# kuldeepbrd1/graspLDM

Hardware: AMD Instinct MI355X
Metric: grasps/sec whole-node (1024-pt cloud, 100 DDIM steps) (higher is better)
Workload: dtype f32 (GEMMs as split-f16 x3 partial products on the f16 matrix pipe, f32 accumulation; GroupNorm / LayerNorm / attention / scheduler in f32); 1 GPU; LDM mode, 256 synthetic 1024-pt clouds per GPU x 20 grasps, 100 DDIM steps: BASELINE.json configs[2] per GPU (configs[3] = this per-GPU workload on 8 GPUs); experiment=fpc, clouds_per_gpu=256, grasps_per_cloud=20, points=1024, ddim_steps=100, encoder=PVCNNEncoder (shipped fpc config), parallelism=cloud-sharded x1, weights=synthetic recipe seed 0, streams=3

## Files before the change

### graspldm_amd/_lib.py

```python
import ctypes
import os

_PKG = os.path.dirname(os.path.abspath(__file__))
LIB_PATH = os.environ.get("GLDM_LIB") or os.path.join(_PKG, "libgldm_hip.so")

ABI_VERSION = 14


class GldmError(RuntimeError):
    pass


_lib = None

_ll = ctypes.c_longlong
_ull = ctypes.c_ulonglong
_vp, _i, _f = ctypes.c_void_p, ctypes.c_int, ctypes.c_float

_SIGNATURES = {
    "gldm_ball_query": [_vp, _vp, _i, _i, _i, _f, _i, _vp, _vp],
    "gldm_grouping_forward": [_vp, _vp, _i, _i, _i, _i, _i, _vp, _vp],
    "gldm_gather_features_forward": [_vp, _vp, _i, _i, _i, _i, _vp, _vp],
    "gldm_furthest_point_sampling": [_vp, _i, _i, _i, _vp, _vp],
    "gldm_three_nn_interpolate_forward": [_vp, _vp, _vp, _i, _i, _i, _i, _vp, _vp, _vp, _vp],
    "gldm_avg_voxelize_forward": [_vp, _vp, _i, _i, _i, _i, _vp, _vp, _vp, _vp],
    "gldm_trilinear_devoxelize_forward": [_vp, _vp, _i, _i, _i, _i, _i, _vp, _vp, _vp, _vp],
    "gldm_voxel_coords": [_vp, _i, _i, _i, _i, _f, _vp, _vp, _vp],
    "gldm_farthest_points_euclid": [_vp, _i, _i, _i, _vp, _vp],
    "gldm_normalize_cloud": [_vp, _i, _i, _f, _f, _f, _f, _f, _f, _vp, _vp, _vp],
    "gldm_gather_points": [_vp, _vp, _i, _i, _i, _vp, _vp],
    "gldm_sa_group": [_vp, _vp, _vp, _i, _i, _i, _i, _f, _i, _vp, _vp, _vp],
    "gldm_r1d_cond_embed": [_vp, _vp, _vp, _i, _i, _i, _i, _vp, _vp],
    "gldm_denoise": [_vp, _vp, _vp, _vp, _i, _vp, _i, _vp, _vp, _i, _i, _i, _vp, _vp, _vp, _vp, _vp, _vp],
    "gldm_denoise_rng": [_vp, _vp, _vp, _vp, _i, _vp, _i, _vp, _i, _i, _vp, _ull, _ll, _vp, _vp, _vp, _vp],
    "gldm_step_noise_rng": [_ull, _ll, _i, _i, _i, _vp, _vp],
    "gldm_decode": [_vp, _vp, _vp, _i, _vp, _i, _vp, _vp, _vp, _vp],
    "gldm_pose_epilogue": [_vp, _vp, _vp, _vp, _i, _i, _i, _vp, _vp, _vp, _vp],
    "gldm_encode": [_vp, _vp, _vp, _i, _vp, _i, _vp, _f, _f, _i, _vp, _vp, _vp, _vp, _vp],
    "gldm_pose_prologue": [_vp, _vp, _vp, _vp, _i, _i, _i, _vp, _vp],
    "gldm_conv3d_k3": [_vp, _vp, _vp, _i, _i, _i, _i, _vp, _vp, _vp],
    "gldm_conv3d_k3_cl": [_vp, _vp, _vp, _i, _i, _i, _i, _vp, _vp, _vp],
    "gldm_conv3d_k3_generic": [_vp, _vp, _vp, _i, _i, _i, _i, _vp, _vp, _vp],
    "gldm_conv3d_k3_f16x2": [_vp, _vp, _vp, _i, _i, _i, _i, _vp, _vp, _vp],
    "gldm_conv3d_k3_f16x2_gn": [_vp, _vp, _vp, _vp, _i, _i, _i, _i, _vp, _vp, _i, _vp],
    "gldm_groupnorm_coef": [_vp, _vp, _vp, _i, _i, _i, _i, _f, _vp, _vp],
    "gldm_gn_swish_chan_sum": [_vp, _vp, _i, _i, _i, _vp, _vp],
    "gldm_gn_swish_chan_sum_cl": [_vp, _vp, _i, _i, _i, _vp, _vp],
    "gldm_se_gate_parts": [_vp, _i, _vp, _vp, _i, _i, _i, _i, _i, _vp, _vp],
    "gldm_groupnorm_swish": [_vp, _vp, _vp, _vp, _i, _i, _i, _i, _f, _vp, _vp],
    "gldm_se_gate": [_vp, _vp, _vp, _i, _i, _i, _i, _i, _vp, _vp],
    "gldm_bias_act": [_vp, _vp, _i, _i, ctypes.c_longlong, _i, _vp],
    "gldm_devoxelize_fused": [_vp, _vp, _vp, _vp, _i, _i, _i, _i, _vp, _vp],
    "gldm_devoxelize_gn_fused": [_vp, _vp, _vp, _vp, _vp, _i, _i, _i, _i, _vp, _vp],
    "gldm_devoxelize_gn_cl_fused": [_vp, _vp, _vp, _vp, _vp, _i, _i, _i, _i, _vp, _vp],
    "gldm_pointwise_mlp": [_vp, _vp, _vp, _i, _i, _i, _i, _i, _vp, _vp, _i, _vp, _vp, _vp],
    "gldm_pointwise_mlp2": [_vp, _vp, _vp, _i, _vp, _vp, _i, _i, _i, _i, _vp, _vp, _i, _vp, _vp, _vp],
    "gldm_pointwise_small": [_vp, _vp, _vp, _i, _i, _i, ctypes.c_longlong, _i, _vp, _vp],
    "gldm_pointwise_any": [_vp, _vp, _vp, _i, _i, _i, ctypes.c_longlong, _i, _vp, _vp],
    "gldm_linear_rows": [_vp, _vp, _vp, _i, _i, _i, _vp, _vp],
    "gldm_pointwise_mlp_f16x2": [_vp, _vp, _vp, _i, _i, _i, _i, _i, _vp, _vp, _i, _vp, _vp, _vp],
    "gldm_row_max": [_vp, _ll, _i, _vp, _vp],
    "gldm_pointwise_mlp_f16x2_pm": [_vp, _vp, _vp, _i, _i, _i, _i, _i, _vp, _vp],
    "gldm_pointwise_mlp_f16x2_add": [_vp, _vp, _vp, _vp, _ll, _ll, _ll, _i, _i, _i, _i, _i, _vp, _vp],
    "gldm_pointwise_mlp2_f16x2": [_vp, _vp, _vp, _i, _vp, _vp, _i, _i, _i, _i, _vp, _vp, _i, _vp, _vp, _vp, _vp],
    "gldm_point_attention": [_vp, _vp, _vp, _i, _i, _i, _i, _vp, _ll, _vp, _vp],
    "gldm_point_attention_workspace_bytes": [_i, _i, _i],
    "gldm_groupnorm_swish_points": [_vp, _vp, _vp, _vp, _i, _i, _i, _i, _f, _vp, _vp],
# ... 76 lines not shown
```

### graspldm_amd/csrc/voxel_conv.hip

```cpp
#include <hip/hip_runtime.h>
#include <stdint.h>
#include <stdio.h>
#include <stdlib.h>

#include "gldm.h"
#include "wstream.h"
#include "devstate.h"

#define GLDM_API extern "C" __attribute__((visibility("default")))

namespace {

using f32x4 = __attribute__((ext_vector_type(4))) float;
typedef __attribute__((address_space(3))) float lds_f;

#ifdef GLDM_DEBUG_KNOBS
__device__ long long g_c3_stamp[32];
#define GLDM_C3_STAMP(i) \
  do { if (blockIdx.x == 5 && blockIdx.y == (gridDim.y >> 1) && threadIdx.x == 0) g_c3_stamp[i] = (long long)__builtin_readcyclecounter(); } while (0)
#else
#define GLDM_C3_STAMP(i) do {} while (0)
#endif

template <int CTRL>
__device__ __forceinline__ float dpp_mov(float x) {
  return __int_as_float(__builtin_amdgcn_update_dpp(0, __float_as_int(x), CTRL, 0xf, 0xf, false));
}
__device__ __forceinline__ float row16_sum(float x) {
  x += dpp_mov<0xB1>(x);
  x += dpp_mov<0x4E>(x);
  x += dpp_mov<0x141>(x);
  x += dpp_mov<0x140>(x);
  return x;
}

constexpr int kConvThreads = 256;
constexpr int kBrick = 4;

__host__ __device__ constexpr bool brick_vec4(int r) { return r <= 24; }
__host__ __device__ constexpr int brick_zp(int r) { return brick_vec4(r) ? r + 8 : r + 2; }
__host__ __device__ constexpr int brick_row_stride(int r) {
  return ((6 * 6 * brick_zp(r) + 31) / 32 * 32 + 16) - 32 >= 6 * 6 * brick_zp(r) ? (6 * 6 * brick_zp(r) + 31) / 32 * 32 - 16
                                                                                 : (6 * 6 * brick_zp(r) + 31) / 32 * 32 + 16;
}

template <int MT, int NTW, int JN>
__global__ __launch_bounds__(kConvThreads, 2) void conv3d_k3_kernel(const float *__restrict__ x,
                                                                    const float *__restrict__ wp,
                                                                    const float *__restrict__ bias, int cin, int cout,
                                                                    int r_arg, float *__restrict__ y,
                                                                    float *__restrict__ partial, int cout_total, int co0,
                                                                    int out_cl) {
  constexpr int r = 4 * NTW;
  (void)r_arg;
  extern __shared__ float lds[];
  __builtin_amdgcn_s_setprio(3);
  GLDM_C3_STAMP(0);
  const int tid = threadIdx.x, wave = tid >> 6, lane = tid & 63;
  const int col = lane & 15, kq = lane >> 4;
  const int bpr = r / kBrick;
// ... 200 lines not shown
#pragma unroll
    for (int mi = 0; mi < MT; ++mi)
#pragma unroll
      for (int q = 0; q < 4; ++q) {
        const int co = 16 * mi + 4 * kq + q;
        if (co < cout) {
#pragma unroll
          for (int ni = 0; ni < NTW; ++ni) y[(size_t)co * r3 + gvox[ni]] = acc[mi][ni][q];
        }
      }
  }
  GLDM_C3_STAMP(21);
}

typedef __attribute__((ext_vector_type(8))) _Float16 c3_f16x8;
typedef __attribute__((ext_vector_type(2))) _Float16 c3_f16x2;
typedef __attribute__((ext_vector_type(2))) float c3_f32x2;
typedef __attribute__((ext_vector_type(4))) unsigned c3_u32x4;
constexpr int kC3Split = 2;

__device__ __forceinline__ void c3_split(const float (&x)[8], c3_u32x4 (&pl)[kC3Split]) {
#pragma unroll
  for (int q = 0; q < 4; ++q) {
    const float a = x[2 * q], b = x[2 * q + 1];
    const c3_f16x2 h = __builtin_convertvector(c3_f32x2{a, b}, c3_f16x2);
    const float ra = __builtin_fmaf((float)h[0], -1.0f, a), rb = __builtin_fmaf((float)h[1], -1.0f, b);
    pl[0][q] = __builtin_bit_cast(unsigned, h);
    pl[1][q] = __builtin_bit_cast(unsigned, __builtin_convertvector(c3_f32x2{ra, rb}, c3_f16x2));
  }
}
__device__ __forceinline__ f32x4 c3_mfma(const c3_u32x4 &a, const c3_u32x4 &b, const f32x4 &c) {
  return __builtin_amdgcn_mfma_f32_16x16x32_f16(__builtin_bit_cast(c3_f16x8, a), __builtin_bit_cast(c3_f16x8, b), c, 0, 0, 0);
}
__device__ __forceinline__ f32x4 c3_mfma3(const c3_u32x4 (&a)[kC3Split], const c3_u32x4 (&b)[kC3Split], f32x4 acc) {
  acc = c3_mfma(a[0], b[1], acc);
  acc = c3_mfma(a[1], b[0], acc);
  return c3_mfma(a[0], b[0], acc);
}

constexpr int kPairs = 14;

__device__ __forceinline__ float c3_range_pow2(float m) {
  int e = (int)((__float_as_uint(m) >> 23) & 0xffu) - 127;
  if ((e >= -8 && e < 14) || e < -100 || e > 100) return 1.0f;
  e = e < -40 ? -40 : e;
  return __uint_as_float((unsigned)(e - 13 + 127) << 23);
}
__device__ __forceinline__ float c3_pow2_inv(float s) { return __uint_as_float((254u << 23) - __float_as_uint(s)); }
__device__ __forceinline__ float c3_wave_max(float x) {
#pragma unroll
  for (int off = 32; off >= 1; off >>= 1) x = fmaxf(x, __shfl_xor(x, off, 64));
  return x;
}

template <int MT, int R, int ZB, int WAVES, bool ACT = false>
__global__ __launch_bounds__(64 * WAVES, (ZB * 16 / WAVES / 16 >= 6) ? 1 : 2) void conv3d_k3_pl_kernel(const float *__restrict__ x,
                                                                                      const float *__restrict__ wp3,
                                                                                      const float *__restrict__ bias, int cin,
                                                                                      int cout, float *__restrict__ y,
                                                                                      float *__restrict__ partial,
                                                                                      const float *__restrict__ in_coef,
                                                                                      int out_cl) {
  constexpr int r = R, NTW = ZB / WAVES, kThreads = 64 * WAVES, kZParts = R / ZB;
  constexpr int GM = MT % 3 == 0 ? 3 : (MT % 4 == 0 ? 4 : (MT % 2 == 0 ? 2 : 1));
  constexpr int GN = NTW % 3 == 0 ? 3 : (NTW % 2 == 0 ? 2 : 1);
  static_assert(R % ZB == 0 && ZB % WAVES == 0, "whole n-tiles per wave");
  constexpr int MG = MT / GM, NG = NTW / GN;
  constexpr int zp = ZB + 2, nvox = 36 * zp, r3 = r * r * r;
  constexpr int hs = (nvox + 15) & ~15;
  constexpr int kItems = 2 * nvox, kRounds = (kItems + kThreads - 1) / kThreads;
  constexpr bool kDB = R == 24 && ZB == 24;
  constexpr bool kRanged = !ACT;
  extern __shared__ float lds[];
  GLDM_C3_STAMP(0);
  __builtin_amdgcn_s_setprio(3);
  const int tid = threadIdx.x, wave = tid >> 6, lane = tid & 63;
  const int col = lane & 15, kq = lane >> 4;
  const int bpr = r / kBrick;
  const int bxy = blockIdx.x / kZParts, bz0 = (blockIdx.x % kZParts) * ZB;
  const int bx0 = (bxy / bpr) * kBrick, by0 = (bxy % bpr) * kBrick;
  const int b = blockIdx.y;
  const int cblocks = (cin + 15) >> 4, kblocks = kPairs * cblocks;
  x += (size_t)b * cin * r3;
  y += (size_t)b * cout * r3;
  const WStream wv(wp3, lane);
  typedef __attribute__((address_space(3))) c3_u32x4 lds_c4;
  constexpr int kSet = kC3Split * 2 * hs;
  lds_c4 *pl0 = (lds_c4 *)lds;

  int vb[NTW];
#pragma unroll
  for (int ni = 0; ni < NTW; ++ni) {
    const int o = 16 * (wave * NTW + ni) + col;
    const int iz = o % ZB, ixy = o / ZB, ix = ixy >> 2, iy = ixy & 3;
    vb[ni] = (ix * 6 + iy) * zp + iz + (kq & 1) * hs;
  }
  f32x4 acc[MT][NTW];
#pragma unroll
  for (int mi = 0; mi < MT; ++mi) {
    f32x4 bvv;
#pragma unroll
    for (int q = 0; q < 4; ++q) bvv[q] = bias[16 * mi + 4 * kq + q];
#pragma unroll
    for (int ni = 0; ni < NTW; ++ni) acc[mi][ni] = bvv;
  }
  int s_lds[kRounds], s_glb[kRounds];
#pragma unroll
  for (int q = 0; q < kRounds; ++q) {
    const int it = tid + q * kThreads;
    s_lds[q] = -1;
    s_glb[q] = -1;
    if (it < kItems) {
      const int h = it / nvox, v = it - h * nvox;
      const int ixy = v / zp, izp = v - ixy * zp;
      const int gx = bx0 + ixy / 6 - 1, gy = by0 + ixy % 6 - 1, gz = bz0 + izp - 1;
      s_lds[q] = h * hs + v;
      if ((unsigned)gx < (unsigned)r && (unsigned)gy < (unsigned)r && (unsigned)gz < (unsigned)r)
        s_glb[q] = (gx * r + gy) * r + gz + 8 * h * r3;
    }
  }
  {
    const c3_u32x4 z4 = c3_u32x4{0u, 0u, 0u, 0u};
#pragma unroll
    for (int q = 0; q < kRounds; ++q)
      if (s_lds[q] >= 0 && s_glb[q] < 0) {
#pragma unroll
        for (int p3 = 0; p3 < kC3Split; ++p3) {
          pl0[p3 * 2 * hs + s_lds[q]] = z4;
          if constexpr (kDB) pl0[kSet + p3 * 2 * hs + s_lds[q]] = z4;
        }
      }
  }
  float stg[kRounds][8];
  auto stage_load = [&](int cb) {
    const float *xc = x + (size_t)(cb * 16) * r3;
#pragma unroll
    for (int q = 0; q < kRounds; ++q) {
      const int g0 = s_glb[q] >= 0 ? s_glb[q] : 0;
#pragma unroll
      for (int j = 0; j < 8; ++j) stg[q][j] = xc[(size_t)j * r3 + g0];
    }
  };
  float *s_coef = lds + (kDB ? 2 : 1) * kSet * 4;
  if constexpr (ACT) {
    for (int i = tid; i < 2 * cin; i += kThreads) s_coef[i] = in_coef[(size_t)b * cin * 2 + i];
  }
  unsigned s_run_u = 0x3f800000u;
  float *rng = s_coef;
  auto stage_store = [&](int cb) {
    lds_c4 *pl = pl0 + (kDB ? (cb & 1) * kSet : 0);
#pragma unroll
    for (int q = 0; q < kRounds; ++q)
      if (s_glb[q] >= 0) {
        if constexpr (kRanged) {
          const float inv_run = __uint_as_float((254u << 23) - s_run_u);
#pragma unroll
          for (int j = 0; j < 8; ++j) stg[q][j] *= inv_run;
        }
        if constexpr (ACT) {
          const int h = (tid + q * kThreads) / nvox;
          const f32x4 *cf = reinterpret_cast<const f32x4 *>(s_coef + 2 * (16 * cb + 8 * h));
#pragma unroll
          for (int j2 = 0; j2 < 4; ++j2) {
// ... 122 lines not shown
      const int co = 16 * mi + 4 * kq + q;
      float s = 0.f, s2 = 0.f;
#pragma unroll
      for (int ni = 0; ni < NTW; ++ni) {
        const float v = acc[mi][ni][q];
        s += v;
        s2 += v * v;
      }
      s = row16_sum(s);
      s2 = row16_sum(s2);
      if (col == 0) {
        s_part[(wave * MT * 16 + co) * 2] = s;
        s_part[(wave * MT * 16 + co) * 2 + 1] = s2;
      }
    }
  }
  __syncthreads();
  if (tid < cout) {
    float s = 0.f, s2 = 0.f;
    for (int w = 0; w < WAVES; ++w) {
      s += s_part[(w * MT * 16 + tid) * 2];
      s2 += s_part[(w * MT * 16 + tid) * 2 + 1];
    }
    float *p = partial + (((size_t)b * (gridDim.x / kZParts) + bxy) * cout + tid) * 2;
    if constexpr (kZParts == 1) {
      p[0] = s;
      p[1] = s2;
    } else {
      atomicAdd(p, s);
      atomicAdd(p + 1, s2);
    }
  }
  int gvox[NTW];
  {
    int lane_o = lane;
    asm volatile("" : "+v"(lane_o));
#pragma unroll
    for (int ni = 0; ni < NTW; ++ni) {
      const int o = 16 * (wave * NTW + ni) + (lane_o & 15);
      const int iz = o % ZB, ixy = o / ZB, ix = ixy >> 2, iy = ixy & 3;
      gvox[ni] = ((bx0 + ix) * r + by0 + iy) * r + bz0 + iz;
    }
  }
  if (out_cl) {
#pragma unroll
    for (int ni = 0; ni < NTW; ++ni)
#pragma unroll
      for (int mi = 0; mi < MT; ++mi)
        *reinterpret_cast<f32x4 *>(y + (size_t)gvox[ni] * cout + 16 * mi + 4 * kq) = acc[mi][ni];
  } else {
#pragma unroll
    for (int mi = 0; mi < MT; ++mi)
#pragma unroll
      for (int q = 0; q < 4; ++q) {
        const int co = 16 * mi + 4 * kq + q;
#pragma unroll
        for (int ni = 0; ni < NTW; ++ni) y[(size_t)co * r3 + gvox[ni]] = acc[mi][ni][q];
      }
  }
  GLDM_C3_STAMP(21);
}

template <int MT, int R, int CIN, int WAVES>
__global__ __launch_bounds__(64 * WAVES, 4) void conv3d_k3_fewch_sp_kernel(const float *__restrict__ x,
                                                                           const float *__restrict__ wp3,
                                                                           const float *__restrict__ bias,
                                                                           float *__restrict__ y,
                                                                           float *__restrict__ partial) {
  constexpr int r = R, NTW = R / WAVES, kThreads = 64 * WAVES, zp = R + 2, nvox = 36 * zp, r3 = r * r * r;
  static_assert(R % WAVES == 0, "whole n-tiles per wave");
  constexpr int K = 27 * CIN, KB = (K + 31) / 32, cout = 16 * MT;
  constexpr int cs = nvox + ((nvox & 31) == 0 ? 8 : 0);
  extern __shared__ float lds[];
  const int tid = threadIdx.x, wave = tid >> 6, lane = tid & 63;
  const int col = lane & 15, g = lane >> 4;
  const int bpr = r / kBrick;
  const int bx0 = (blockIdx.x / bpr) * kBrick, by0 = (blockIdx.x % bpr) * kBrick;
  const int b = blockIdx.y;
  x += (size_t)b * CIN * r3;
  y += (size_t)b * cout * r3;
  float mx = 0.f;
  for (int i = tid; i < CIN * nvox; i += kThreads) {
    const int ci = i / nvox, v = i - ci * nvox;
    const int ixy = v / zp, izp = v - ixy * zp;
    const int gx = bx0 + ixy / 6 - 1, gy = by0 + ixy % 6 - 1, gz = izp - 1;
    float val = 0.f;
    if ((unsigned)gx < (unsigned)r && (unsigned)gy < (unsigned)r && (unsigned)gz < (unsigned)r)
      val = x[(size_t)ci * r3 + (gx * r + gy) * r + gz];
    lds[ci * cs + v] = val;
    mx = fmaxf(mx, fabsf(val));
  }
  float *rng = lds + CIN * cs;
  mx = c3_wave_max(mx);
  if (lane == 0) rng[wave] = mx;
  int vb[NTW], gvox[NTW];
#pragma unroll
  for (int ni = 0; ni < NTW; ++ni) {
    const int o = 16 * (wave * NTW + ni) + col;
    const int iz = o % r, ixy = o / r, ix = ixy >> 2, iy = ixy & 3;
    vb[ni] = (ix * 6 + iy) * zp + iz;
    gvox[ni] = ((bx0 + ix) * r + by0 + iy) * r + iz;
// ... 62 lines not shown
      const int co = 16 * mi + 4 * g + q;
      float s = 0.f, s2 = 0.f;
#pragma unroll
      for (int ni = 0; ni < NTW; ++ni) {
        const float v = acc[mi][ni][q];
        s += v;
        s2 += v * v;
      }
      s = row16_sum(s);
      s2 = row16_sum(s2);
      if (col == 0) {
        s_part[(wave * MT * 16 + co) * 2] = s;
        s_part[(wave * MT * 16 + co) * 2 + 1] = s2;
      }
    }
  }
  __syncthreads();
  if (tid < cout) {
    float s = 0.f, s2 = 0.f;
    for (int w = 0; w < WAVES; ++w) {
      s += s_part[(w * MT * 16 + tid) * 2];
      s2 += s_part[(w * MT * 16 + tid) * 2 + 1];
    }
    float *p = partial + (((size_t)b * gridDim.x + blockIdx.x) * cout + tid) * 2;
    p[0] = s;
    p[1] = s2;
  }
#pragma unroll
  for (int mi = 0; mi < MT; ++mi)
#pragma unroll
    for (int q = 0; q < 4; ++q) {
      const int co = 16 * mi + 4 * g + q;
#pragma unroll
      for (int ni = 0; ni < NTW; ++ni) y[(size_t)co * r3 + gvox[ni]] = acc[mi][ni][q];
    }
}

__global__ __launch_bounds__(512) void groupnorm_swish_kernel(float *__restrict__ y, const float *__restrict__ partial,
                                                              const float *__restrict__ gamma,
                                                              const float *__restrict__ beta, int c, int r3,
                                                              int nbricks, int groups, float eps,
                                                              float *__restrict__ chan_sum) {
  __shared__ double s_stat[2];
  __shared__ float s_red[8];
  const int g = blockIdx.x, b = blockIdx.y, cpg = c / groups;
  const int tid = threadIdx.x;
  if (tid < 64) {
    double s = 0.0, s2 = 0.0;
    for (int i = tid; i < nbricks * cpg; i += 64) {
      const int br = i / cpg, ch = g * cpg + i % cpg;
      const float *p = partial + (((size_t)b * nbricks + br) * c + ch) * 2;
      s += (double)p[0];
      s2 += (double)p[1];
    }
    for (int off = 32; off >= 1; off >>= 1) {
      s += __shfl_xor(s, off, 64);
      s2 += __shfl_xor(s2, off, 64);
    }
// ... 487 lines not shown
  GLDM_CONV_CASE(2, 4);
  GLDM_CONV_CASE(4, 2);
  GLDM_CONV_CASE(1, 4);
  GLDM_CONV_CASE(2, 2);
  GLDM_CONV_CASE(4, 1);
  GLDM_CONV_CASE(8, 1);
#undef GLDM_CONV_CASE
  if (mt == 4 && ntw == 8) return launch_conv_halves<2, 8>(x, w_packed, bias, b, cin, cout, r, y, partial, s, out_cl);
  if (mt == 16 && ntw == 2) return launch_conv_halves<8, 2>(x, w_packed, bias, b, cin, cout, r, y, partial, s, out_cl);
  if (mt == 8 && ntw == 4) return launch_conv_halves<4, 4>(x, w_packed, bias, b, cin, cout, r, y, partial, s, out_cl);
  return GLDM_ERR_UNSUPPORTED;
}

GLDM_API int gldm_conv3d_k3(const float *x, const float *w_packed, const float *bias, int b, int cin, int cout, int r,
                            float *y, float *partial, gldm_stream_t stream) {
  return conv3d_k3_impl(x, w_packed, bias, b, cin, cout, r, y, partial, 0, stream);
}

GLDM_API int gldm_conv3d_k3_cl(const float *x, const float *w_packed, const float *bias, int b, int cin, int cout, int r,
                               float *y_cl, float *partial, gldm_stream_t stream) {
  return conv3d_k3_impl(x, w_packed, bias, b, cin, cout, r, y_cl, partial, 1, stream);
}

template <int MT, int R, int ZB, int WAVES, bool ACT>
int launch_conv_pl_act(const float *x, const float *wp3, const float *bias, int b, int cin, int cout, float *y, float *partial,
                       const float *in_coef, int out_cl, hipStream_t s) {
  const size_t lds_bytes = (size_t)(R == 24 && ZB == 24 ? 2 : 1) * kC3Split * 2 * ((36 * (ZB + 2) + 15) & ~15) * 16 +
                           (ACT ? (size_t)2 * cin * sizeof(float) : 64 );
  struct Tag {};
  gldm_dev::allow_dynamic_lds<Tag>(reinterpret_cast<const void *>(&conv3d_k3_pl_kernel<MT, R, ZB, WAVES, ACT>), (int)lds_bytes);
  const int bpr = R / kBrick;
  if (R != ZB) {
    if (hipMemsetAsync(partial, 0, (size_t)b * bpr * bpr * cout * 2 * sizeof(float), s) != hipSuccess) return GLDM_ERR_LAUNCH;
  }
  hipLaunchKernelGGL((conv3d_k3_pl_kernel<MT, R, ZB, WAVES, ACT>), dim3(bpr * bpr * (R / ZB), b), dim3(64 * WAVES), lds_bytes,
                     s, x, wp3, bias, cin, cout, y, partial, in_coef, out_cl);
  return hipGetLastError() == hipSuccess ? GLDM_OK : GLDM_ERR_LAUNCH;
}
template <int MT, int R, int ZB, int WAVES>
int launch_conv_pl(const float *x, const float *wp3, const float *bias, int b, int cin, int cout, float *y, float *partial,
                   const float *in_coef, int out_cl, hipStream_t s) {
  return in_coef ? launch_conv_pl_act<MT, R, ZB, WAVES, true>(x, wp3, bias, b, cin, cout, y, partial, in_coef, out_cl, s)
                 : launch_conv_pl_act<MT, R, ZB, WAVES, false>(x, wp3, bias, b, cin, cout, y, partial, nullptr, out_cl, s);
}

static int conv3d_k3_f16x2_impl(const float *x, const float *in_coef, const float *w_split, const float *bias, int b, int cin,
                                 int cout, int r, float *y, float *partial, int out_cl, gldm_stream_t stream) {
  if (!x || !w_split || !bias || !y || !partial || b <= 0 || cin <= 0 || cout <= 0 || r <= 0) return GLDM_ERR_INVALID_ARG;
  if ((in_coef || out_cl) && cin % 16) return GLDM_ERR_UNSUPPORTED;
  hipStream_t s = reinterpret_cast<hipStream_t>(stream);
  if (cin == 3 && cout == 48 && r == 24) {
    constexpr int kZp = 26, kNvox = 36 * kZp;
    const size_t lds_bytes = (size_t)3 * (kNvox + ((kNvox & 31) == 0 ? 8 : 0)) * sizeof(float) + 64;
    hipLaunchKernelGGL((conv3d_k3_fewch_sp_kernel<3, 24, 3, 8>), dim3(36, b), dim3(512), lds_bytes, s, x, w_split, bias, y, partial);
    return hipGetLastError() == hipSuccess ? GLDM_OK : GLDM_ERR_LAUNCH;
  }
  if (cin % 16) return GLDM_ERR_UNSUPPORTED;
#ifdef GLDM_DEBUG_KNOBS
  struct StampDump {
    hipStream_t s; int cin, cout, r, b;
    ~StampDump() {
      if (!getenv("GLDM_C3_STAMP")) return;
      long long h[32];
      (void)hipStreamSynchronize(s);
      (void)hipMemcpyFromSymbol(h, HIP_SYMBOL(g_c3_stamp), sizeof(h));
      printf("conv3d split %d->%d @%d b=%d: setup %lld, stage0 issue %lld", cin, cout, r, b, h[1] - h[0], h[2] - h[1]);
      for (int cb = 0; cb < cin / 16 && cb < 3; ++cb)
        printf(" | cb%d: wait %lld store %lld barrier %lld taps %lld", cb, h[3 + 4 * cb] - (cb ? h[2 + 4 * cb] : h[2]),
               h[4 + 4 * cb] - h[3 + 4 * cb], h[5 + 4 * cb] - h[4 + 4 * cb], h[6 + 4 * cb] - h[5 + 4 * cb]);
      printf(" | epilogue %lld, total %lld\n", h[21] - h[20], h[21] - h[0]);
    }
  } dump{s, cin, cout, r, b};
#endif
  if (cout == 48 && r == 24) return launch_conv_pl<3, 24, 24, 8>(x, w_split, bias, b, cin, cout, y, partial, in_coef, out_cl, s);
  if (cout == 96 && r == 12) return launch_conv_pl<6, 12, 12, 4>(x, w_split, bias, b, cin, cout, y, partial, in_coef, out_cl, s);
  if (cout == 32 && r == 32) return launch_conv_pl<2, 32, 32, 8>(x, w_split, bias, b, cin, cout, y, partial, in_coef, out_cl, s);
  if (cout == 64 && r == 32) return launch_conv_pl<4, 32, 32, 8>(x, w_split, bias, b, cin, cout, y, partial, in_coef, out_cl, s);
  if (cout == 32 && r == 16) return launch_conv_pl<2, 16, 16, 4>(x, w_split, bias, b, cin, cout, y, partial, in_coef, out_cl, s);
  if (cout == 64 && r == 16) return launch_conv_pl<4, 16, 16, 4>(x, w_split, bias, b, cin, cout, y, partial, in_coef, out_cl, s);
  if (cout == 128 && r == 16) return launch_conv_pl<8, 16, 16, 8>(x, w_split, bias, b, cin, cout, y, partial, in_coef, out_cl, s);
  if (cout == 64 && r == 8) return launch_conv_pl<4, 8, 8, 4>(x, w_split, bias, b, cin, cout, y, partial, in_coef, out_cl, s);
  if (cout == 128 && r == 8) return launch_conv_pl<8, 8, 8, 4>(x, w_split, bias, b, cin, cout, y, partial, in_coef, out_cl, s);
  if (cout == 256 && r == 8) return launch_conv_pl<16, 8, 8, 8>(x, w_split, bias, b, cin, cout, y, partial, in_coef, out_cl, s);
  if (cout == 128 && r == 4) return launch_conv_pl<8, 4, 4, 4>(x, w_split, bias, b, cin, cout, y, partial, in_coef, out_cl, s);
  return GLDM_ERR_UNSUPPORTED;
}

GLDM_API int gldm_conv3d_k3_f16x2(const float *x, const float *w_split, const float *bias, int b, int cin, int cout, int r,
                                   float *y, float *partial, gldm_stream_t stream) {
  return conv3d_k3_f16x2_impl(x, nullptr, w_split, bias, b, cin, cout, r, y, partial, 0, stream);
}

GLDM_API int gldm_conv3d_k3_f16x2_gn(const float *x, const float *in_coef, const float *w_split, const float *bias, int b,
                                      int cin, int cout, int r, float *y, float *partial, int out_channel_last,
                                      gldm_stream_t stream) {
  return conv3d_k3_f16x2_impl(x, in_coef, w_split, bias, b, cin, cout, r, y, partial, out_channel_last ? 1 : 0, stream);
}

GLDM_API int gldm_groupnorm_coef(const float *partial, const float *gamma, const float *beta, int b, int c, int r, int groups,
                                 float eps, float *coef, gldm_stream_t stream) {
  if (!partial || !gamma || !beta || !coef || b <= 0 || c <= 0 || r <= 0 || groups <= 0 || c % groups || c / groups > 128)
    return GLDM_ERR_INVALID_ARG;
  const int nbricks = ((r + kBrick - 1) / kBrick) * ((r + kBrick - 1) / kBrick);
  hipLaunchKernelGGL(groupnorm_coef_kernel, dim3(groups, b), dim3(64), 0, reinterpret_cast<hipStream_t>(stream), partial, gamma,
                     beta, c, r * r * r, nbricks, groups, eps, coef);
  return hipGetLastError() == hipSuccess ? GLDM_OK : GLDM_ERR_LAUNCH;
}

GLDM_API int gldm_gn_swish_chan_sum(const float *y, const float *coef, int b, int c, int r, float *chan_sum,
                                    gldm_stream_t stream) {
  if (!y || !coef || !chan_sum || b <= 0 || c <= 0 || r <= 0) return GLDM_ERR_INVALID_ARG;
  hipLaunchKernelGGL(gn_swish_sum_kernel, dim3(c, b), dim3(256), 0, reinterpret_cast<hipStream_t>(stream), y, coef, c,
                     r * r * r, chan_sum);
  return hipGetLastError() == hipSuccess ? GLDM_OK : GLDM_ERR_LAUNCH;
}

GLDM_API int gldm_groupnorm_swish(float *y, const float *partial, const float *gamma, const float *beta, int b, int c,
                                  int r, int groups, float eps, float *chan_sum, gldm_stream_t stream) {
  if (!y || !partial || !gamma || !beta || b <= 0 || c <= 0 || r <= 0 || groups <= 0 || c % groups)
    return GLDM_ERR_INVALID_ARG;
  const int nbricks = ((r + kBrick - 1) / kBrick) * ((r + kBrick - 1) / kBrick);
// ... 110 lines not shown
```

### graspldm_amd/voxel.py

```python
import torch

from . import _lib as L
from .r1d_pack import mfma_a_fragments

SUPPORTED = {(3, 6), (6, 3), (2, 8), (4, 4), (8, 2), (4, 8), (2, 4), (4, 2), (1, 4), (2, 2), (4, 1), (8, 1),
             (16, 2), (8, 4)}


SPLIT_SHAPES = {(48, 24), (96, 12), (32, 32), (64, 32), (32, 16), (64, 16), (128, 16), (64, 8), (128, 8), (256, 8), (128, 4)}


def conv_supported(cout, r):
    return cout % 16 == 0 and r % 4 == 0 and (cout // 16, r // 4) in SUPPORTED


def pack_conv3d(weight):
    cout, cin = weight.shape[:2]
    cpad = (cin + 15) // 16 * 16
    w = torch.zeros(cout, 27, cpad, dtype=torch.float32)
    w[:, :, :cin] = weight.detach().float().cpu().reshape(cout, cin, 27).permute(0, 2, 1)
    return mfma_a_fragments(w.reshape(cout, 27 * cpad))


def split_conv_supported(cin, cout, r):
# ... 24 lines not shown
    taps = torch.zeros(cout, cb, 16, 28)
    taps[..., :27] = wt
    w[:] = taps.reshape(cout, cb, 16, 14, 2).permute(0, 1, 3, 4, 2)
    return mfma_a_fragments_f16x2(w.reshape(cout, cb * 14 * 32))


class VoxelBranchPlan:

    def __init__(self, convs, device, r=None):
        from .r1d_pack import SplitRangeError
        self.split = [r is not None and split_conv_supported(c.in_channels, c.out_channels, r) for c in convs]
        self.generic = [r is not None and not conv_supported(c.out_channels, r) for c in convs]
        self.w = []
        for i, c in enumerate(convs):
            if self.split[i]:
                try:
                    self.w.append((pack_conv3d_fewch_f16x2(c.weight) if c.in_channels < 16 else pack_conv3d_f16x2(c.weight)).to(device))
                    continue
                except SplitRangeError:
                    self.split[i] = False
            self.w.append((c.weight.detach().float().contiguous() if self.generic[i] else pack_conv3d(c.weight)).to(device))


def _launch_conv(plan, i, conv, x, coef, b, r, cl, st):
    cin, cout = conv.in_channels, conv.out_channels
    y = torch.empty((b, cout, r, r, r), dtype=torch.float32, device=x.device)
    nf = L.lib().gldm_conv3d_partial_floats(b, cout, r)
    partial = torch.empty(int(nf), dtype=torch.float32, device=x.device)
    staged = plan.split[i] and cin % 16 == 0
    if staged and (coef is not None or cl):
        L.call("gldm_conv3d_k3_f16x2_gn", L.ptr(x), L.ptr(coef), L.ptr(plan.w[i]), L.ptr(conv.bias), b, cin, cout, r,
               L.ptr(y), L.ptr(partial), 1 if cl else 0, st)
    elif cl:
        assert coef is None
        L.call("gldm_conv3d_k3_cl", L.ptr(x), L.ptr(plan.w[i]), L.ptr(conv.bias), b, cin, cout, r, L.ptr(y), L.ptr(partial), st)
    else:
        assert coef is None
        entry = "gldm_conv3d_k3_generic" if plan.generic[i] else ("gldm_conv3d_k3_f16x2" if plan.split[i] else "gldm_conv3d_k3")
        L.call(entry, L.ptr(x), L.ptr(plan.w[i]), L.ptr(conv.bias), b, cin, cout, r, L.ptr(y), L.ptr(partial), st)
    return y, partial


def _next_conv_stages_norm(plan, convs, i, r):
    return plan.split[i + 1] and convs[i + 1].in_channels % 16 == 0 and r >= 16


def _groupnorm_coef(partial, gn, b, c, r, st):
    coef = torch.empty((b, c, 2), dtype=torch.float32, device=partial.device)
    L.call("gldm_groupnorm_coef", L.ptr(partial), L.ptr(gn.weight), L.ptr(gn.bias), b, c, r, gn.num_groups, float(gn.eps),
           L.ptr(coef), st)
    return coef


def run(plan, convs, norms, se, vox, norm_coords, point_feat, r):
    dev = vox.device
    b = vox.shape[0]
    st = L.current_stream(dev)
    x = vox.contiguous()
    coef = None
    chan_sum = None
    x_cl = False
    with torch.cuda.device(dev):
        for i, (conv, gn) in enumerate(zip(convs, norms)):
            cin, cout = conv.in_channels, conv.out_channels
            last = i == len(convs) - 1
            staged = plan.split[i] and cin % 16 == 0
            mfma32 = not plan.split[i] and not plan.generic[i]
            cl = last and (staged or mfma32) and cout % 4 == 0 and cout <= 256 and cout // gn.num_groups <= 64
            y, partial = _launch_conv(plan, i, conv, x, coef, b, r, cl, st)
            x_cl = cl
            foldable = (last or _next_conv_stages_norm(plan, convs, i, r)) and cout // gn.num_groups <= 64
            if foldable:
                coef = _groupnorm_coef(partial, gn, b, cout, r, st)
            else:
                coef = None
                if last and se is not None:
                    chan_sum = torch.empty((b, cout), dtype=torch.float32, device=dev)
                L.call("gldm_groupnorm_swish", L.ptr(y), L.ptr(partial), L.ptr(gn.weight), L.ptr(gn.bias), b, cout, r,
                       gn.num_groups, float(gn.eps), L.ptr(chan_sum) if (last and se is not None) else None, st)
            x = y
        c = x.shape[1]
        gate = None
        if se is not None:
            gate = torch.empty((b, c), dtype=torch.float32, device=dev)
            w1, w2 = se.fc[0].weight, se.fc[2].weight
            if x_cl:
                parts = int(L.lib().gldm_squeeze_parts())
                chan_sum = torch.empty((b, parts, c), dtype=torch.float32, device=dev)
                L.call("gldm_gn_swish_chan_sum_cl", L.ptr(x), L.ptr(coef), b, c, r, L.ptr(chan_sum), st)
                L.call("gldm_se_gate_parts", L.ptr(chan_sum), parts, L.ptr(w1), L.ptr(w2), b, c, w1.shape[0], r,
                       1 if se.use_relu else 0, L.ptr(gate), st)
            else:
                if coef is not None:
                    chan_sum = torch.empty((b, c), dtype=torch.float32, device=dev)
# ... 1 lines not shown
                L.call("gldm_se_gate", L.ptr(chan_sum), L.ptr(w1), L.ptr(w2), b, c, w1.shape[0], r,
                       1 if se.use_relu else 0, L.ptr(gate), st)
        n = norm_coords.shape[2]
        out = torch.empty((b, c, n), dtype=torch.float32, device=dev)
        pf = point_feat.contiguous() if point_feat is not None else None
        if x_cl:
            L.call("gldm_devoxelize_gn_cl_fused", L.ptr(norm_coords), L.ptr(x), L.ptr(coef), L.ptr(gate), L.ptr(pf), b, c, n, r,
                   L.ptr(out), st)
        elif coef is not None:
            L.call("gldm_devoxelize_gn_fused", L.ptr(norm_coords), L.ptr(x), L.ptr(coef), L.ptr(gate), L.ptr(pf), b, c, n, r,
                   L.ptr(out), st)
        else:
            L.call("gldm_devoxelize_fused", L.ptr(norm_coords), L.ptr(x), L.ptr(gate), L.ptr(pf), b, c, n, r, L.ptr(out), st)
    return out


def run_attention(plan, convs, norms, attn, se, vox, norm_coords, point_feat, r):
    from . import attention as A
    dev = vox.device
    b = vox.shape[0]
    st = L.current_stream(dev)
    x = vox.contiguous()
    coef = None
    with torch.cuda.device(dev):
        for i, (conv, gn) in enumerate(zip(convs, norms)):
            cout, last = conv.out_channels, i == len(convs) - 1
            y, partial = _launch_conv(plan, i, conv, x, coef, b, r, False, st)
            if last or (_next_conv_stages_norm(plan, convs, i, r) and cout // gn.num_groups <= 64):
                coef = _groupnorm_coef(partial, gn, b, cout, r, st)
            else:
                coef = None
                L.call("gldm_groupnorm_swish", L.ptr(y), L.ptr(partial), L.ptr(gn.weight), L.ptr(gn.bias), b, cout, r,
                       gn.num_groups, float(gn.eps), None, st)
            x = y
        c = x.shape[1]
        xa = torch.empty((b, c, r ** 3), dtype=torch.float32, device=dev)
        L.call("gldm_groupnorm_affine", L.ptr(x), L.ptr(coef), b, c, r, L.ptr(xa), st)
        pq, po = attn._packed(dev)
        h = A.run_conv(A.attention_core(A.run_conv(xa, pq), xa, xa), po)
        gate = None
        if se is not None:
            feat, chan_sum = A.groupnorm_swish_sum(h, attn.norm, add=xa)
            gate = torch.empty((b, c), dtype=torch.float32, device=dev)
            w1, w2 = se.fc[0].weight, se.fc[2].weight
            L.call("gldm_se_gate", L.ptr(chan_sum), L.ptr(w1), L.ptr(w2), b, c, w1.shape[0], r, 1 if se.use_relu else 0,
                   L.ptr(gate), st)
        else:
            feat = A.groupnorm_swish(h, attn.norm, add=xa)
        n = norm_coords.shape[2]
        out = torch.empty((b, c, n), dtype=torch.float32, device=dev)
# ... 4 lines not shown
```

### include/gldm.h

```cpp
#ifndef GLDM_H_
#define GLDM_H_

#include <stdint.h>

#ifdef __cplusplus
extern "C" {
#endif

typedef void *gldm_stream_t;

enum gldm_status {
  GLDM_OK = 0,
  GLDM_ERR_INVALID_ARG = -1,
  GLDM_ERR_LAUNCH = -2,
  GLDM_ERR_UNSUPPORTED = -3,
  GLDM_ERR_WORKSPACE = -4
};

int gldm_abi_version(void);
const char *gldm_status_string(int status);


int gldm_ball_query(const float *centers , const float *points ,
                    int b, int n, int m, float radius, int u,
// ... 201 lines not shown


long long gldm_conv3d_partial_floats(int b, int cout, int r);
int gldm_conv3d_k3(const float *x , const float *w_packed, const float *bias ,
                   int b, int cin, int cout, int r, float *y , float *partial,
                   gldm_stream_t stream);

int gldm_conv3d_k3_cl(const float *x , const float *w_packed, const float *bias , int b, int cin,
                      int cout, int r, float *y_cl , float *partial, gldm_stream_t stream);

int gldm_conv3d_k3_generic(const float *x , const float *w , const float *bias,
                           int b, int cin, int cout, int r, float *y , float *partial,
                           gldm_stream_t stream);

int gldm_conv3d_k3_f16x2(const float *x , const float *w_split, const float *bias ,
                          int b, int cin, int cout, int r, float *y , float *partial,
                          gldm_stream_t stream);

int gldm_conv3d_k3_f16x2_gn(const float *x , const float *in_coef ,
                             const float *w_split, const float *bias , int b, int cin, int cout, int r,
                             float *y , float *partial, int out_channel_last,
                             gldm_stream_t stream);

int gldm_groupnorm_coef(const float *partial, const float *gamma, const float *beta, int b, int c, int r, int groups,
                        float eps, float *coef , gldm_stream_t stream);

int gldm_gn_swish_chan_sum(const float *y , const float *coef , int b, int c, int r,
                           float *chan_sum , gldm_stream_t stream);

int gldm_squeeze_parts(void);
int gldm_gn_swish_chan_sum_cl(const float *y , const float *coef , int b, int c, int r,
                              float *chan_parts , gldm_stream_t stream);

int gldm_groupnorm_swish(float *y , const float *partial, const float *gamma, const float *beta,
                         int b, int c, int r, int groups, float eps, float *chan_sum, gldm_stream_t stream);

int gldm_se_gate(const float *chan_sum , const float *w1 , const float *w2 ,
                 int b, int c, int hidden, int r, int use_relu, float *gate , gldm_stream_t stream);
int gldm_se_gate_parts(const float *chan_parts , int parts, const float *w1, const float *w2, int b, int c,
                       int hidden, int r, int use_relu, float *gate , gldm_stream_t stream);

int gldm_devoxelize_fused(const float *coords , const float *features ,
                          const float *gate , const float *add , int b, int c, int n, int r,
                          float *out , gldm_stream_t stream);

int gldm_devoxelize_gn_fused(const float *coords , const float *features ,
// ... 48 lines not shown
```

Before: 312,000 grasps/s.

## Use 8-channel blocked voxel layout between r=24 convs and XCD-aware block ordering

Adds a channel-blocked-by-8 voxel layout for intermediates between consecutive 48-channel r=24 3D convolutions. The consumer can then gather 8 channels with two 16-byte vector loads instead of eight strided scalar loads, and the producer writes them with vector stores. It also flattens the grid and remaps block indices so each XCD works on a contiguous range of clouds, which should improve L2 locality. Separately, FP contraction is disabled in the f16 split routine to keep the residual exact. The blocked path adds layout constraints and alignment checks, and it only applies to specific shapes.

```diff
diff --git a/graspldm_amd/_lib.py b/graspldm_amd/_lib.py
--- a/graspldm_amd/_lib.py
+++ b/graspldm_amd/_lib.py
@@ -43,6 +43,7 @@
     "gldm_conv3d_k3_generic": [_vp, _vp, _vp, _i, _i, _i, _i, _vp, _vp, _vp],
     "gldm_conv3d_k3_f16x2": [_vp, _vp, _vp, _i, _i, _i, _i, _vp, _vp, _vp],
     "gldm_conv3d_k3_f16x2_gn": [_vp, _vp, _vp, _vp, _i, _i, _i, _i, _vp, _vp, _i, _vp],
+    "gldm_conv3d_k3_f16x2_blk": [_vp, _vp, _vp, _vp, _i, _i, _i, _i, _vp, _vp, _i, _i, _vp],
     "gldm_groupnorm_coef": [_vp, _vp, _vp, _i, _i, _i, _i, _f, _vp, _vp],
     "gldm_gn_swish_chan_sum": [_vp, _vp, _i, _i, _i, _vp, _vp],
     "gldm_gn_swish_chan_sum_cl": [_vp, _vp, _i, _i, _i, _vp, _vp],
diff --git a/graspldm_amd/csrc/voxel_conv.hip b/graspldm_amd/csrc/voxel_conv.hip
--- a/graspldm_amd/csrc/voxel_conv.hip
+++ b/graspldm_amd/csrc/voxel_conv.hip
@@ -36,6 +36,17 @@
 
 constexpr int kConvThreads = 256;
 constexpr int kBrick = 4;
+
+constexpr int kVoxCM = 0, kVoxCL = 1, kVoxBlk8 = 2;
+
+__device__ __forceinline__ int xcd_work_item(int wg, int total) {
+  const int x = wg & 7, q = total >> 3, rem = total & 7;
+  return x * q + (x < rem ? x : rem) + (wg >> 3);
+}
+#ifndef GLDM_XCD_MIN_CLOUDS
+#define GLDM_XCD_MIN_CLOUDS 1
+#endif
+constexpr int kXcdMinClouds = GLDM_XCD_MIN_CLOUDS;
 
 __host__ __device__ constexpr bool brick_vec4(int r) { return r <= 24; }
 __host__ __device__ constexpr int brick_zp(int r) { return brick_vec4(r) ? r + 8 : r + 2; }
@@ -282,6 +293,7 @@
 __device__ __forceinline__ void c3_split(const float (&x)[8], c3_u32x4 (&pl)[kC3Split]) {
 #pragma unroll
   for (int q = 0; q < 4; ++q) {
+#pragma clang fp contract(off)
     const float a = x[2 * q], b = x[2 * q + 1];
     const c3_f16x2 h = __builtin_convertvector(c3_f32x2{a, b}, c3_f16x2);
     const float ra = __builtin_fmaf((float)h[0], -1.0f, a), rb = __builtin_fmaf((float)h[1], -1.0f, b);
@@ -313,14 +325,14 @@
   return x;
 }
 
-template <int MT, int R, int ZB, int WAVES, bool ACT = false>
+template <int MT, int R, int ZB, int WAVES, bool ACT = false, bool BLK = false>
 __global__ __launch_bounds__(64 * WAVES, (ZB * 16 / WAVES / 16 >= 6) ? 1 : 2) void conv3d_k3_pl_kernel(const float *__restrict__ x,
                                                                                       const float *__restrict__ wp3,
                                                                                       const float *__restrict__ bias, int cin,
                                                                                       int cout, float *__restrict__ y,
                                                                                       float *__restrict__ partial,
                                                                                       const float *__restrict__ in_coef,
-                                                                                      int out_cl) {
+                                                                                      int out_cl, int xcd_order) {
   constexpr int r = R, NTW = ZB / WAVES, kThreads = 64 * WAVES, kZParts = R / ZB;
   constexpr int GM = MT % 3 == 0 ? 3 : (MT % 4 == 0 ? 4 : (MT % 2 == 0 ? 2 : 1));
   constexpr int GN = NTW % 3 == 0 ? 3 : (NTW % 2 == 0 ? 2 : 1);
@@ -336,10 +348,15 @@
   __builtin_amdgcn_s_setprio(3);
   const int tid = threadIdx.x, wave = tid >> 6, lane = tid & 63;
   const int col = lane & 15, kq = lane >> 4;
-  const int bpr = r / kBrick;
-  const int bxy = blockIdx.x / kZParts, bz0 = (blockIdx.x % kZParts) * ZB;
+  constexpr int bpr = r / kBrick, kBricks = bpr * bpr * kZParts;
+  int brick = blockIdx.x, b = blockIdx.y;
+  if (xcd_order) {
+    const int item = xcd_work_item((int)blockIdx.x, (int)gridDim.x);
+    b = item / kBricks;
+    brick = item - b * kBricks;
+  }
+  const int bxy = brick / kZParts, bz0 = (brick % kZParts) * ZB;
   const int bx0 = (bxy / bpr) * kBrick, by0 = (bxy % bpr) * kBrick;
-  const int b = blockIdx.y;
   const int cblocks = (cin + 15) >> 4, kblocks = kPairs * cblocks;
   x += (size_t)b * cin * r3;
   y += (size_t)b * cout * r3;
@@ -376,7 +393,7 @@
       const int gx = bx0 + ixy / 6 - 1, gy = by0 + ixy % 6 - 1, gz = bz0 + izp - 1;
       s_lds[q] = h * hs + v;
       if ((unsigned)gx < (unsigned)r && (unsigned)gy < (unsigned)r && (unsigned)gz < (unsigned)r)
-        s_glb[q] = (gx * r + gy) * r + gz + 8 * h * r3;
+        s_glb[q] = BLK ? ((gx * r + gy) * r + gz + h * r3) * 8 : (gx * r + gy) * r + gz + 8 * h * r3;
     }
   }
   {
@@ -397,8 +414,17 @@
 #pragma unroll
     for (int q = 0; q < kRounds; ++q) {
       const int g0 = s_glb[q] >= 0 ? s_glb[q] : 0;
-#pragma unroll
-      for (int j = 0; j < 8; ++j) stg[q][j] = xc[(size_t)j * r3 + g0];
+      if constexpr (BLK) {
+        const f32x4 lo = *reinterpret_cast<const f32x4 *>(xc + g0), hi = *reinterpret_cast<const f32x4 *>(xc + g0 + 4);
+#pragma unroll
+        for (int j = 0; j < 4; ++j) {
+          stg[q][j] = lo[j];
+          stg[q][4 + j] = hi[j];
+        }
+      } else {
+#pragma unroll
+        for (int j = 0; j < 8; ++j) stg[q][j] = xc[(size_t)j * r3 + g0];
+      }
     }
   };
   float *s_coef = lds + (kDB ? 2 : 1) * kSet * 4;
@@ -567,7 +593,7 @@
       s += s_part[(w * MT * 16 + tid) * 2];
       s2 += s_part[(w * MT * 16 + tid) * 2 + 1];
     }
-    float *p = partial + (((size_t)b * (gridDim.x / kZParts) + bxy) * cout + tid) * 2;
+    float *p = partial + (((size_t)b * (bpr * bpr) + bxy) * cout + tid) * 2;
     if constexpr (kZParts == 1) {
       p[0] = s;
       p[1] = s2;
@@ -587,7 +613,13 @@
       gvox[ni] = ((bx0 + ix) * r + by0 + iy) * r + bz0 + iz;
     }
   }
-  if (out_cl) {
+  if (out_cl == kVoxBlk8) {
+#pragma unroll
+    for (int mi = 0; mi < MT; ++mi)
+#pragma unroll
+      for (int ni = 0; ni < NTW; ++ni)
+        *reinterpret_cast<f32x4 *>(y + ((size_t)(2 * mi + (kq >> 1)) * r3 + gvox[ni]) * 8 + 4 * (kq & 1)) = acc[mi][ni];
+  } else if (out_cl) {
 #pragma unroll
     for (int ni = 0; ni < NTW; ++ni)
 #pragma unroll
@@ -611,7 +643,8 @@
                                                                            const float *__restrict__ wp3,
                                                                            const float *__restrict__ bias,
                                                                            float *__restrict__ y,
-                                                                           float *__restrict__ partial) {
+                                                                           float *__restrict__ partial, int out_blk,
+                                                                           int xcd_order) {
   constexpr int r = R, NTW = R / WAVES, kThreads = 64 * WAVES, zp = R + 2, nvox = 36 * zp, r3 = r * r * r;
   static_assert(R % WAVES == 0, "whole n-tiles per wave");
   constexpr int K = 27 * CIN, KB = (K + 31) / 32, cout = 16 * MT;
@@ -619,9 +652,14 @@
   extern __shared__ float lds[];
   const int tid = threadIdx.x, wave = tid >> 6, lane = tid & 63;
   const int col = lane & 15, g = lane >> 4;
-  const int bpr = r / kBrick;
-  const int bx0 = (blockIdx.x / bpr) * kBrick, by0 = (blockIdx.x % bpr) * kBrick;
-  const int b = blockIdx.y;
+  constexpr int bpr = r / kBrick, kBricks = bpr * bpr;
+  int brick = blockIdx.x, b = blockIdx.y;
+  if (xcd_order) {
+    const int item = xcd_work_item((int)blockIdx.x, (int)gridDim.x);
+    b = item / kBricks;
+    brick = item - b * kBricks;
+  }
+  const int bx0 = (brick / bpr) * kBrick, by0 = (brick % bpr) * kBrick;
   x += (size_t)b * CIN * r3;
   y += (size_t)b * cout * r3;
   float mx = 0.f;
@@ -730,18 +768,26 @@
       s += s_part[(w * MT * 16 + tid) * 2];
       s2 += s_part[(w * MT * 16 + tid) * 2 + 1];
     }
-    float *p = partial + (((size_t)b * gridDim.x + blockIdx.x) * cout + tid) * 2;
+    float *p = partial + (((size_t)b * kBricks + brick) * cout + tid) * 2;
     p[0] = s;
     p[1] = s2;
   }
-#pragma unroll
-  for (int mi = 0; mi < MT; ++mi)
-#pragma unroll
-    for (int q = 0; q < 4; ++q) {
-      const int co = 16 * mi + 4 * g + q;
-#pragma unroll
-      for (int ni = 0; ni < NTW; ++ni) y[(size_t)co * r3 + gvox[ni]] = acc[mi][ni][q];
-    }
+  if (out_blk) {
+#pragma unroll
+    for (int mi = 0; mi < MT; ++mi)
+#pragma unroll
+      for (int ni = 0; ni < NTW; ++ni)
+        *reinterpret_cast<f32x4 *>(y + ((size_t)(2 * mi + (g >> 1)) * r3 + gvox[ni]) * 8 + 4 * (g & 1)) = acc[mi][ni];
+  } else {
+#pragma unroll
+    for (int mi = 0; mi < MT; ++mi)
+#pragma unroll
+      for (int q = 0; q < 4; ++q) {
+        const int co = 16 * mi + 4 * g + q;
+#pragma unroll
+        for (int ni = 0; ni < NTW; ++ni) y[(size_t)co * r3 + gvox[ni]] = acc[mi][ni][q];
+      }
+  }
 }
 
 __global__ __launch_bounds__(512) void groupnorm_swish_kernel(float *__restrict__ y, const float *__restrict__ partial,
@@ -1275,37 +1321,47 @@
   return conv3d_k3_impl(x, w_packed, bias, b, cin, cout, r, y_cl, partial, 1, stream);
 }
 
-template <int MT, int R, int ZB, int WAVES, bool ACT>
+template <int MT, int R, int ZB, int WAVES, bool ACT, bool BLK = false>
 int launch_conv_pl_act(const float *x, const float *wp3, const float *bias, int b, int cin, int cout, float *y, float *partial,
                        const float *in_coef, int out_cl, hipStream_t s) {
   const size_t lds_bytes = (size_t)(R == 24 && ZB == 24 ? 2 : 1) * kC3Split * 2 * ((36 * (ZB + 2) + 15) & ~15) * 16 +
                            (ACT ? (size_t)2 * cin * sizeof(float) : 64 );
   struct Tag {};
-  gldm_dev::allow_dynamic_lds<Tag>(reinterpret_cast<const void *>(&conv3d_k3_pl_kernel<MT, R, ZB, WAVES, ACT>), (int)lds_bytes);
+  gldm_dev::allow_dynamic_lds<Tag>(reinterpret_cast<const void *>(&conv3d_k3_pl_kernel<MT, R, ZB, WAVES, ACT, BLK>), (int)lds_bytes);
   const int bpr = R / kBrick;
   if (R != ZB) {
     if (hipMemsetAsync(partial, 0, (size_t)b * bpr * bpr * cout * 2 * sizeof(float), s) != hipSuccess) return GLDM_ERR_LAUNCH;
   }
-  hipLaunchKernelGGL((conv3d_k3_pl_kernel<MT, R, ZB, WAVES, ACT>), dim3(bpr * bpr * (R / ZB), b), dim3(64 * WAVES), lds_bytes,
-                     s, x, wp3, bias, cin, cout, y, partial, in_coef, out_cl);
+  const int bricks = bpr * bpr * (R / ZB);
+  const bool xcd = R == 24 && b >= kXcdMinClouds;
+  hipLaunchKernelGGL((conv3d_k3_pl_kernel<MT, R, ZB, WAVES, ACT, BLK>), xcd ? dim3(bricks * b) : dim3(bricks, b), dim3(64 * WAVES),
+                     lds_bytes, s, x, wp3, bias, cin, cout, y, partial, in_coef, out_cl, xcd ? 1 : 0);
   return hipGetLastError() == hipSuccess ? GLDM_OK : GLDM_ERR_LAUNCH;
 }
-template <int MT, int R, int ZB, int WAVES>
+template <int MT, int R, int ZB, int WAVES, bool BLK = false>
 int launch_conv_pl(const float *x, const float *wp3, const float *bias, int b, int cin, int cout, float *y, float *partial,
                    const float *in_coef, int out_cl, hipStream_t s) {
-  return in_coef ? launch_conv_pl_act<MT, R, ZB, WAVES, true>(x, wp3, bias, b, cin, cout, y, partial, in_coef, out_cl, s)
-                 : launch_conv_pl_act<MT, R, ZB, WAVES, false>(x, wp3, bias, b, cin, cout, y, partial, nullptr, out_cl, s);
+  return in_coef ? launch_conv_pl_act<MT, R, ZB, WAVES, true, BLK>(x, wp3, bias, b, cin, cout, y, partial, in_coef, out_cl, s)
+                 : launch_conv_pl_act<MT, R, ZB, WAVES, false, BLK>(x, wp3, bias, b, cin, cout, y, partial, nullptr, out_cl, s);
 }
 
 static int conv3d_k3_f16x2_impl(const float *x, const float *in_coef, const float *w_split, const float *bias, int b, int cin,
-                                 int cout, int r, float *y, float *partial, int out_cl, gldm_stream_t stream) {
+                                 int cout, int r, float *y, float *partial, int out_cl, gldm_stream_t stream,
+                                 int in_layout = kVoxCM) {
   if (!x || !w_split || !bias || !y || !partial || b <= 0 || cin <= 0 || cout <= 0 || r <= 0) return GLDM_ERR_INVALID_ARG;
-  if ((in_coef || out_cl) && cin % 16) return GLDM_ERR_UNSUPPORTED;
+  if (out_cl != kVoxCM && out_cl != kVoxCL && out_cl != kVoxBlk8) return GLDM_ERR_INVALID_ARG;
+  if (in_layout != kVoxCM && in_layout != kVoxBlk8) return GLDM_ERR_INVALID_ARG;
+  if ((in_layout == kVoxBlk8 || out_cl == kVoxBlk8) && !(cout == 48 && r == 24)) return GLDM_ERR_UNSUPPORTED;
+  if (in_layout == kVoxBlk8 && (cin % 16 || ((uintptr_t)x & 15))) return GLDM_ERR_UNSUPPORTED;
+  if (out_cl == kVoxBlk8 && ((uintptr_t)y & 15)) return GLDM_ERR_UNSUPPORTED;
+  if ((in_coef || out_cl == kVoxCL) && cin % 16) return GLDM_ERR_UNSUPPORTED;
   hipStream_t s = reinterpret_cast<hipStream_t>(stream);
   if (cin == 3 && cout == 48 && r == 24) {
     constexpr int kZp = 26, kNvox = 36 * kZp;
     const size_t lds_bytes = (size_t)3 * (kNvox + ((kNvox & 31) == 0 ? 8 : 0)) * sizeof(float) + 64;
-    hipLaunchKernelGGL((conv3d_k3_fewch_sp_kernel<3, 24, 3, 8>), dim3(36, b), dim3(512), lds_bytes, s, x, w_split, bias, y, partial);
+    const bool xcd = b >= kXcdMinClouds;
+    hipLaunchKernelGGL((conv3d_k3_fewch_sp_kernel<3, 24, 3, 8>), xcd ? dim3(36 * b) : dim3(36, b), dim3(512), lds_bytes, s, x,
+                       w_split, bias, y, partial, out_cl == kVoxBlk8 ? 1 : 0, xcd ? 1 : 0);
     return hipGetLastError() == hipSuccess ? GLDM_OK : GLDM_ERR_LAUNCH;
   }
   if (cin % 16) return GLDM_ERR_UNSUPPORTED;
@@ -1325,6 +1381,8 @@
     }
   } dump{s, cin, cout, r, b};
 #endif
+  if (cout == 48 && r == 24 && in_layout == kVoxBlk8)
+    return launch_conv_pl<3, 24, 24, 8, true>(x, w_split, bias, b, cin, cout, y, partial, in_coef, out_cl, s);
   if (cout == 48 && r == 24) return launch_conv_pl<3, 24, 24, 8>(x, w_split, bias, b, cin, cout, y, partial, in_coef, out_cl, s);
   if (cout == 96 && r == 12) return launch_conv_pl<6, 12, 12, 4>(x, w_split, bias, b, cin, cout, y, partial, in_coef, out_cl, s);
   if (cout == 32 && r == 32) return launch_conv_pl<2, 32, 32, 8>(x, w_split, bias, b, cin, cout, y, partial, in_coef, out_cl, s);
@@ -1350,6 +1408,12 @@
   return conv3d_k3_f16x2_impl(x, in_coef, w_split, bias, b, cin, cout, r, y, partial, out_channel_last ? 1 : 0, stream);
 }
 
+GLDM_API int gldm_conv3d_k3_f16x2_blk(const float *x, const float *in_coef, const float *w_split, const float *bias, int b,
+                                       int cin, int cout, int r, float *y, float *partial, int in_layout, int out_layout,
+                                       gldm_stream_t stream) {
+  return conv3d_k3_f16x2_impl(x, in_coef, w_split, bias, b, cin, cout, r, y, partial, out_layout, stream, in_layout);
+}
+
 GLDM_API int gldm_groupnorm_coef(const float *partial, const float *gamma, const float *beta, int b, int c, int r, int groups,
                                  float eps, float *coef, gldm_stream_t stream) {
   if (!partial || !gamma || !beta || !coef || b <= 0 || c <= 0 || r <= 0 || groups <= 0 || c % groups || c / groups > 128)
diff --git a/graspldm_amd/voxel.py b/graspldm_amd/voxel.py
--- a/graspldm_amd/voxel.py
+++ b/graspldm_amd/voxel.py
@@ -70,13 +70,22 @@
             self.w.append((c.weight.detach().float().contiguous() if self.generic[i] else pack_conv3d(c.weight)).to(device))
 
 
-def _launch_conv(plan, i, conv, x, coef, b, r, cl, st):
+VOX_CM, VOX_CL, VOX_BLK8 = 0, 1, 2
+
+BLOCKED_INTERMEDIATE = True
+
+
+def _launch_conv(plan, i, conv, x, coef, b, r, cl, st, x_blk=False, y_blk=False):
     cin, cout = conv.in_channels, conv.out_channels
     y = torch.empty((b, cout, r, r, r), dtype=torch.float32, device=x.device)
     nf = L.lib().gldm_conv3d_partial_floats(b, cout, r)
     partial = torch.empty(int(nf), dtype=torch.float32, device=x.device)
     staged = plan.split[i] and cin % 16 == 0
-    if staged and (coef is not None or cl):
+    if x_blk or y_blk:
+        assert plan.split[i] and not (cl and y_blk)
+        L.call("gldm_conv3d_k3_f16x2_blk", L.ptr(x), L.ptr(coef), L.ptr(plan.w[i]), L.ptr(conv.bias), b, cin, cout, r,
+               L.ptr(y), L.ptr(partial), VOX_BLK8 if x_blk else VOX_CM, VOX_BLK8 if y_blk else (VOX_CL if cl else VOX_CM), st)
+    elif staged and (coef is not None or cl):
         L.call("gldm_conv3d_k3_f16x2_gn", L.ptr(x), L.ptr(coef), L.ptr(plan.w[i]), L.ptr(conv.bias), b, cin, cout, r,
                L.ptr(y), L.ptr(partial), 1 if cl else 0, st)
     elif cl:
@@ -93,6 +102,14 @@
     return plan.split[i + 1] and convs[i + 1].in_channels % 16 == 0 and r >= 16
 
 
+def _blocked_between(plan, convs, norms, i, r):
+    if not BLOCKED_INTERMEDIATE or i + 1 >= len(convs) or r != 24:
+        return False
+    a, c = convs[i], convs[i + 1]
+    return (plan.split[i] and (a.in_channels == 3 or a.in_channels % 16 == 0) and a.out_channels == 48 and c.out_channels == 48
+            and _next_conv_stages_norm(plan, convs, i, r) and a.out_channels // norms[i].num_groups <= 64)
+
+
 def _groupnorm_coef(partial, gn, b, c, r, st):
     coef = torch.empty((b, c, 2), dtype=torch.float32, device=partial.device)
     L.call("gldm_groupnorm_coef", L.ptr(partial), L.ptr(gn.weight), L.ptr(gn.bias), b, c, r, gn.num_groups, float(gn.eps),
@@ -108,6 +125,7 @@
     coef = None
     chan_sum = None
     x_cl = False
+    x_blk = False
     with torch.cuda.device(dev):
         for i, (conv, gn) in enumerate(zip(convs, norms)):
             cin, cout = conv.in_channels, conv.out_channels
@@ -115,9 +133,11 @@
             staged = plan.split[i] and cin % 16 == 0
             mfma32 = not plan.split[i] and not plan.generic[i]
             cl = last and (staged or mfma32) and cout % 4 == 0 and cout <= 256 and cout // gn.num_groups <= 64
-            y, partial = _launch_conv(plan, i, conv, x, coef, b, r, cl, st)
-            x_cl = cl
+            y_blk = _blocked_between(plan, convs, norms, i, r)
+            y, partial = _launch_conv(plan, i, conv, x, coef, b, r, cl, st, x_blk, y_blk)
+            x_cl, x_blk = cl, y_blk
             foldable = (last or _next_conv_stages_norm(plan, convs, i, r)) and cout // gn.num_groups <= 64
+            assert foldable or not y_blk
             if foldable:
                 coef = _groupnorm_coef(partial, gn, b, cout, r, st)
             else:
@@ -165,10 +185,13 @@
     st = L.current_stream(dev)
     x = vox.contiguous()
     coef = None
+    x_blk = False
     with torch.cuda.device(dev):
         for i, (conv, gn) in enumerate(zip(convs, norms)):
             cout, last = conv.out_channels, i == len(convs) - 1
-            y, partial = _launch_conv(plan, i, conv, x, coef, b, r, False, st)
+            y_blk = _blocked_between(plan, convs, norms, i, r)
+            y, partial = _launch_conv(plan, i, conv, x, coef, b, r, False, st, x_blk, y_blk)
+            x_blk = y_blk
             if last or (_next_conv_stages_norm(plan, convs, i, r) and cout // gn.num_groups <= 64):
                 coef = _groupnorm_coef(partial, gn, b, cout, r, st)
             else:
diff --git a/include/gldm.h b/include/gldm.h
--- a/include/gldm.h
+++ b/include/gldm.h
@@ -247,6 +247,13 @@
                              float *y , float *partial, int out_channel_last,
                              gldm_stream_t stream);
 
+#define GLDM_VOX_CM 0
+#define GLDM_VOX_CL 1
+#define GLDM_VOX_BLK8 2
+int gldm_conv3d_k3_f16x2_blk(const float *x, const float *in_coef , const float *w_split,
+                              const float *bias , int b, int cin, int cout, int r, float *y, float *partial,
+                              int in_layout, int out_layout, gldm_stream_t stream);
+
 int gldm_groupnorm_coef(const float *partial, const float *gamma, const float *beta, int b, int c, int r, int groups,
                         float eps, float *coef , gldm_stream_t stream);
 
```

Measured after the change: 313,500 grasps/s (median of 6 runs). No clear change (+0.5%).
